# Z-Zheng/ever

Measured on AMD Instinct MI355X. Metric: 512x512 tiles/sec fwd+bwd, FarSeg-R50, higher is better.
Workload: dtype f32; 1 GPU; FarSeg ResNet-50 FPN (FarSegHead defaults, BCE+dice), 3-band 512x512, batch 16/GPU, fwd+bwd+SGD step, inputs resident in HBM; global_batch=16, parallelism=single

## Files before the change

### ever_amd/_C.py

```python
import ctypes as C
import os

_LIB_PATH = os.path.join(os.path.dirname(os.path.abspath(__file__)), 'lib', 'libever_hip.so')
_LIB_PATH = os.environ.get('EVK_LIB', _LIB_PATH)

c_void_p, c_int, c_i32, c_i64, c_u32, c_f32, c_size_t = (
    C.c_void_p, C.c_int, C.c_int32, C.c_int64, C.c_uint32, C.c_float, C.c_size_t)


class ConvDesc(C.Structure):
    _fields_ = [(n, c_i32) for n in (
        'N', 'H', 'W', 'Cin', 'Ho', 'Wo', 'Cout', 'kh', 'kw',
        'stride_h', 'stride_w', 'pad_h', 'pad_w', 'dil_h', 'dil_w')]


class SplitJob(C.Structure):
    _fields_ = [('w', c_void_p), ('out', c_void_p), ('kind', c_i32), ('arg', c_i32 * 13)]


P = c_void_p
_DP = C.POINTER(ConvDesc)
_JP = C.POINTER(SplitJob)

SIGNATURES = {
# ... 58 lines not shown
    'evk_bn_plan': (c_int, [c_i64, c_i32, c_i32, C.POINTER(c_i32)]),
    'evk_bn_fwd_train': (c_int, [P, P, P, P, P, P, c_f32, c_f32, P, P, P, c_i64, c_i32, c_u32, P, c_size_t, P, P]),
    'evk_bn_fwd_train_parts': (c_int, [P, P, P, P, P, P, c_f32, c_f32, P, P, P, c_i64, c_i32, c_u32, P, c_i32, P, c_size_t, P, P]),
    'evk_bn_fwd_train_parts_bits': (c_int, [P, P, P, P, P, P, c_f32, c_f32, P, P, P, c_i64, c_i32, c_u32, P, c_i32, P, c_size_t, P, P, P]),
    'evk_relu_bits_bytes': (c_size_t, [c_i64]),
    'evk_relu_bits_apply': (c_int, [P, P, P, c_i64, P]),
    'evk_bn_fwd_eval': (c_int, [P, P, P, P, P, P, c_f32, P, P, P, c_i64, c_i32, c_u32, P, c_size_t, P, P]),
    'evk_bn_relu_pool_fwd_train_parts': (c_int, [P, P, P, P, P, c_f32, c_f32, P, P, P, P, c_i32, c_i32, c_i32, c_i32, P, c_i32,
                                                 P, c_size_t, P, P]),
    'evk_bn_relu_pool_bwd': (c_int, [P, P, P, P, P, P, P, P, P, P, c_i32, c_i32, c_i32, c_i32, c_i32, P, c_size_t, P, P]),
    'evk_bn_bwd': (c_int, [P, P, P, P, P, P, P, P, P, P, P, c_i64, c_i32, c_u32, c_i32, P, c_size_t, P, P]),
    'evk_stream_fork': (c_int, [P, P]),
    'evk_streams_overlap': (c_int, [P, P, c_i32, P]),
    'evk_bn_relu_dot_fwd': (c_int, [P, P, P, P, P, c_i64, c_i32, c_i32, P]),
    'evk_bn_relu_dot_workspace_bytes': (c_size_t, [c_i64, c_i32, c_i32]),
    'evk_bn_relu_dot_bwd': (c_int, [P, P, P, P, P, P, P, P, P, P, P, P, c_i64, c_i32, c_i32, c_u32, P, c_size_t, P, P]),
    'evk_bn_finalize_parts': (c_int, [P, c_i32, c_i32, c_i64, P, P, P, P, c_f32, c_f32, P, P, P, P]),
    'evk_relation_bn_fwd': (c_int, [P, P, P, P, P, P, P, c_i32, c_i32, c_i32, P, P]),
    'evk_relation_bn_parts': (c_i32, [c_i32, c_i32]),
    'evk_relation_bn_workspace_bytes': (c_size_t, [c_i32, c_i32, c_i32]),
    'evk_relation_bn_bwd': (c_int, [P, P, P, P, P, P, P, P, P, P, P, P, c_i32, c_i32, c_i32, P, c_size_t, P]),
    'evk_bn_bwd_from_partials': (c_int, [P, P, P, P, P, P, P, c_i32, P, P, P, c_i64, c_i32, c_u32, c_i32, P, c_size_t, P, P]),
    'evk_bn_bwd_bits': (c_int, [P, P, P, P, P, P, P, P, P, P, P, c_i64, c_i32, c_u32, c_i32, P, c_size_t, P, P, P]),
    'evk_relu_fwd': (c_int, [P, P, c_i64, P]),
    'evk_relu_bwd': (c_int, [P, P, P, c_i64, P]),
    'evk_add': (c_int, [P, P, P, c_i64, P]),
    'evk_scale': (c_int, [P, c_f32, P, c_i64, P]),
    'evk_group_weight_expand': (c_int, [P, P, c_i32, c_i32, c_i32, c_i32, P]),
    'evk_group_weight_gather': (c_int, [P, P, c_i32, c_i32, c_i32, c_i32, P]),
    'evk_mul_scale': (c_int, [P, P, c_f32, P, c_i64, P]),
    'evk_gelu_fwd': (c_int, [P, P, c_i64, P]),
    'evk_gelu_bwd': (c_int, [P, P, P, c_i64, P]),
    'evk_maxpool3x3s2_fwd': (c_int, [P, P, P, c_i32, c_i32, c_i32, c_i32, P]),
    'evk_maxpool3x3s2_bwd': (c_int, [P, P, P, c_i32, c_i32, c_i32, c_i32, P]),
    'evk_upsample_nearest2x_add_fwd': (c_int, [P, P, P, c_i32, c_i32, c_i32, c_i32, P, P]),
    'evk_upsample_nearest2x_bwd': (c_int, [P, P, c_i32, c_i32, c_i32, c_i32, P]),
    'evk_subsample2_fwd': (c_int, [P, P, c_i32, c_i32, c_i32, c_i32, P]),
    'evk_subsample2_bwd': (c_int, [P, P, c_i32, c_i32, c_i32, c_i32, P]),
    'evk_upsample_bilinear_fwd': (c_int, [P, P, c_i32, c_i32, c_i32, c_i32, c_i32, c_i32, P]),
    'evk_upsample_bilinear_bwd': (c_int, [P, P, c_i32, c_i32, c_i32, c_i32, c_i32, c_i32, P]),
    'evk_upsample_bilinear_plan': (c_int, [c_i32, c_i32, c_i32, c_i32, c_i32, c_i32, c_i32, c_i32, C.POINTER(c_i32)]),
    'evk_upsample_bilinear_slice_fwd': (c_int, [P, P, c_i32, c_i32, c_i32, c_i32, c_i32, c_i32, c_i32, c_i32, P]),
    'evk_upsample_bilinear_slice_bwd': (c_int, [P, P, c_i32, c_i32, c_i32, c_i32, c_i32, c_i32, c_i32, c_i32, P]),
    'evk_hr_fuse_fwd': (c_int, [P, P, P, c_i32, P, P, P, c_i32, c_i32, c_i32, c_i32, P]),
    'evk_hr_fuse_bwd': (c_int, [P, P, P, P, P, P, c_i32, c_i32, c_i32, c_i32, P]),
    'evk_wfuse_fwd': (c_int, [P, P, c_i32, P, c_i32, c_f32, P, c_i32, c_i32, c_i32, c_i32, P]),
# ... 103 lines not shown
```

### ever_amd/csrc/bn.hip

```cpp
#include "bn_common.hpp"

namespace evk {

__global__ __launch_bounds__(256) void bn_stats_partial_kernel(const float* __restrict__ x, float* __restrict__ partial,
                                                               int64_t rows, int C, int64_t rows_per_blk, int tpc,
                                                               int rl) {
  __shared__ f32x4 red[2][256];
  const int c4 = C >> 2;
  const int tc = threadIdx.x % tpc, tr = threadIdx.x / tpc;
  const int64_t r0 = (int64_t)blockIdx.x * rows_per_blk;
  const int64_t r1 = min(rows, r0 + rows_per_blk);
  for (int cb = tc; cb < c4; cb += tpc) {
    f32x4 s = {0.f, 0.f, 0.f, 0.f}, q = {0.f, 0.f, 0.f, 0.f};
    const f32x4 pv = *reinterpret_cast<const f32x4*>(x + cb * 4);
    if (tr < rl) {
      int64_t r = r0 + tr;
      const int64_t st = rl;
      for (; r + 3 * st < r1; r += 4 * st) {
        const f32x4 v0 = *reinterpret_cast<const f32x4*>(x + r * C + cb * 4) - pv;
        const f32x4 v1 = *reinterpret_cast<const f32x4*>(x + (r + st) * C + cb * 4) - pv;
        const f32x4 v2 = *reinterpret_cast<const f32x4*>(x + (r + 2 * st) * C + cb * 4) - pv;
        const f32x4 v3 = *reinterpret_cast<const f32x4*>(x + (r + 3 * st) * C + cb * 4) - pv;
        s += (v0 + v1) + (v2 + v3);
        q += (v0 * v0 + v1 * v1) + (v2 * v2 + v3 * v3);
// ... 698 lines not shown
  hipLaunchKernelGGL(bn_bwd_sums_final_kernel, dim3((C + kFinCh - 1) / kFinCh), dim3(256), 0, st, (const float*)partial,
                     pl.nblk, C, sums);
  return check_launch("bn_bwd_local_sums");
}

extern "C" int evk_bn_bwd_apply_sums(const float* dy, const float* x, const float* y, const float* gamma,
                                     const float* beta, const float* mean, const float* invstd, const float* mean_g,
                                     const float* mean_gx, float* dx, int64_t rows, int32_t C, uint32_t flags,
                                     void* workspace, size_t workspace_bytes, void* stream) {
  EVK_REQUIRE(dy && x && mean && invstd && mean_g && mean_gx && dx, EVK_E_INVALID, "bn_bwd_apply_sums: null pointer");
  const int relu = (flags & EVK_BN_RELU) ? (y ? 1 : 2) : 0;
  int rc = bn_check("bn_bwd_apply_sums", rows, C, workspace, workspace_bytes, BnWorkspace::bytes(C));
  if (rc) return rc;
  hipStream_t st = (hipStream_t)stream;
  float* coef = (float*)workspace;
  hipLaunchKernelGGL(bn_bwd_coef_kernel, dim3((C + 255) / 256), dim3(256), 0, st, gamma, invstd, mean_g, mean_gx, C, coef);
  rc = check_launch("bn_bwd_coef");
  if (rc) return rc;
  const size_t n4 = (size_t)rows * C / 4;
  hipLaunchKernelGGL(bn_bwd_apply_kernel<false>, dim3(oneshot_grid(n4)), dim3(256), 0, st, dy, x, y, mean,
                     invstd, (const float*)coef, gamma, beta, dx, n4, C, relu, (uint32_t*)nullptr);
  return check_launch("bn_bwd_apply_sums");
}
```

### ever_amd/csrc/bn_common.hpp

```cpp
#pragma once
#include "x3_common.hpp"

namespace evk {

__device__ __forceinline__ unsigned bn_blk() { return gridDim.x - 1u - blockIdx.x; }

__device__ __forceinline__ int bn_fin_group() { return xcd_remap((int)blockIdx.x, (int)gridDim.x); }

__device__ __forceinline__ f32x4 bn_ld(const float* p, size_t i) {
  return __builtin_nontemporal_load(reinterpret_cast<const f32x4*>(p) + i);
}

constexpr int kMaxStatBlocks = 2048;

__device__ __forceinline__ void zero_amax(uint32_t* __restrict__ amax) {
  if (amax && blockIdx.x == 0 && threadIdx.x < kAmaxSlots) amax[threadIdx.x * kAmaxStride] = 0;
}

struct BnPlan {
  int nblk;
  int64_t rows_per_blk;
  int tpc, rl;
};
inline BnPlan bn_plan(int64_t rows, int C, int64_t per_override = 0, int64_t cap_override = 0) {
// ... 47 lines not shown
__device__ __forceinline__ f32x4 relu_mask(f32x4 g, const f32x4 yy) {
  g.x = yy.x > 0.f ? g.x : 0.f; g.y = yy.y > 0.f ? g.y : 0.f;
  g.z = yy.z > 0.f ? g.z : 0.f; g.w = yy.w > 0.f ? g.w : 0.f;
  return g;
}

__device__ __forceinline__ void fold_store_record(f32x4 (*red)[256], f32x4 s, f32x4 q, float* rec, size_t blk, int C, int cb,
                                                  int tc, int tr, int tpc, int rl) {
  red[0][threadIdx.x] = s;
  red[1][threadIdx.x] = q;
  __syncthreads();
  if (tr == 0) {
    for (int k = 1; k < rl; ++k) {
      s += red[0][k * tpc + tc];
      q += red[1][k * tpc + tc];
    }
    float* o = rec + blk * 2 * C;
    *reinterpret_cast<f32x4*>(o + cb * 4) = s;
    *reinterpret_cast<f32x4*>(o + C + cb * 4) = q;
  }
  __syncthreads();
}

constexpr int kFinCh = 8;
template <int FC, typename T, typename Op>
__device__ __forceinline__ T fold_channel_lanes(T v, T (*lds)[FC], Op op) {
#pragma unroll
  for (int o = FC; o < 64; o <<= 1) v = op(v, __shfl_xor(v, o, 64));
  const int lane = threadIdx.x & 63, w = threadIdx.x >> 6;
  if (lane < FC) lds[w][lane] = v;
  __syncthreads();
  const int tc = threadIdx.x % FC;
  const T r = op(op(lds[0][tc], lds[1][tc]), op(lds[2][tc], lds[3][tc]));
  __syncthreads();
  return r;
}
template <int FC = kFinCh>
__device__ __forceinline__ bool reduce_partials(const float* __restrict__ partial, int nblk, int C, int& c, double& s,
                                                double& q) {
  __shared__ double red[4][FC];
  const int tc = threadIdx.x % FC, tl = threadIdx.x / FC;
  c = bn_fin_group() * FC + tc;
  s = 0.0;
  q = 0.0;
  if (c < C) {
    const float* ps = partial + c;
// ... 47 lines not shown
```

### ever_amd/hip/_base.py

```python
import ctypes
import os

import torch
from torch.autograd import Function
from torch.autograd.function import once_differentiable

from .. import _C
from . import timing, weight_planes
from .workspace import workspace


class HipPathError(RuntimeError):
    """Raised when the HIP path is asked to run on something it cannot (CPU tensor, wrong dtype)."""


_CONV_MATH = os.environ.get('EVK_CONV_MATH', 'f16x2')
_MATH_MODES = ('f16x2', 'bf16x3', 'f32', 'bf16')


def _planes_math():
    return _CONV_MATH in ('f16x2', 'bf16x3', 'bf16')


def _f16x2():
# ... 114 lines not shown
    import torch.distributed as dist
    return dist.is_available() and dist.is_initialized()


def _collectives_world():
    import torch.distributed as dist
    return dist.get_world_size() if _dist_initialized() else 1


def _mark_packed(t, bits):
    _note_amax(t, bits)
    t._evk_packed = (t._version, t.data_ptr())
    absmax_stats['packed'] += 1
    return t


def _is_packed(t):
    hit = getattr(t, '_evk_packed', None)
    return hit is not None and hit[0] == t._version and hit[1] == t.data_ptr()


_RELU_BITS = os.environ.get('EVK_RELU_BITS', '1') != '0'
_LAZY_RES = os.environ.get('EVK_LAZY_RES', '1') != '0'
relu_bits_stats = {'forward': 0, 'lazy': 0, 'masked_dgrad': 0, 'masked_bn': 0, 'materialized': 0}


def _lazy_bits(t):
    hit = getattr(t, '_evk_relu_bits', None)
    if hit is not None and hit[0] == t._version and hit[1] == t.data_ptr():
        return hit[2]
    return None


def materialize_lazy(t):
    bits = _lazy_bits(t) if t is not None else None
    if bits is None:
        return t
    out = torch.empty_like(t)
    _C.call('evk_relu_bits_apply', t.data_ptr(), bits.data_ptr(), out.data_ptr(), t.numel(), _stream())
    relu_bits_stats['materialized'] += 1
    return _inherit_amax(out, t)


_top_saved_hooks = getattr(torch._C._autograd, '_top_saved_tensors_default_hooks', None)


def observers_active():
# ... 94 lines not shown
```

### ever_amd/hip/norm.py

```python
import ctypes
import os

import torch
from torch.autograd import Function
from torch.autograd.function import once_differentiable

from .. import _C
from . import timing, weight_planes
from .workspace import workspace
from ._base import (
    HipPathError, _AMAX_HANDOFF, _LAZY_RES, _PACKED, _RELU_BITS, _amax_out, _amax_zeroed, _f16x2, _inherit_amax,
    _lazy_bits, _mark_packed, _note_amax, _ptr, _require_cuda, _stream, _timed_call, as_nhwc, empty_nhwc, materialize_lazy,
    observers_active, relu_bits_stats,
)


class _BatchNormActFn(Function):

    @staticmethod
    def forward(ctx, x, residual, weight, bias, running_mean, running_var, training, momentum, eps, relu, parts=None,
                pack_out=False, lazy_res=False):
        n, c, h, w = x.shape
        rows = n * h * w
        dev = x.device
        st = _stream()
        lib = _C.load()
        ws_bytes = lib.evk_bn_workspace_bytes(rows, c)
        ws = workspace(dev, ws_bytes)
        y = empty_nhwc(n, c, h, w, dev)
        save_mean = torch.empty((c,), device=dev, dtype=torch.float32)
        save_invstd = torch.empty((c,), device=dev, dtype=torch.float32)
        flags = 1 if relu else 0
        pack = bool(pack_out and _PACKED and _f16x2() and training and parts is not None and residual is None
                    and c % 8 == 0 and rows >= 256 and not observers_active())
        abits = _amax_zeroed(dev) if pack else _amax_out(dev)
# ... 88 lines not shown
    if x.shape[1] % 4 != 0:
        raise HipPathError(f'batch_norm: channel count {x.shape[1]} must be a multiple of 4')
    if residual is not None:
        residual = as_nhwc(residual, 'batch_norm.residual')
    use_batch_stats = training or running_mean is None
    parts = getattr(x, '_evk_bn_parts', None) if use_batch_stats else None
    if parts is not None:
        del x._evk_bn_parts
    _AMAX_HANDOFF[0] = None
    if use_batch_stats and running_mean is not None:
        weight_planes.note_running_stats_changed()
    y = _BatchNormActFn.apply(x, residual, weight, bias, running_mean, running_var, bool(use_batch_stats),
                              0.0 if momentum is None else momentum, eps, bool(relu), parts, bool(pack_out), bool(lazy_res))
    if _AMAX_HANDOFF[0] is not None:
        abits, packed = _AMAX_HANDOFF[0]
        if packed:
            _mark_packed(y, abits)
        elif abits is not None:
            _note_amax(y, abits)
        _AMAX_HANDOFF[0] = None
    return y


class _BnReluPoolFn(Function):

    @staticmethod
    def forward(ctx, x, weight, bias, running_mean, running_var, momentum, eps, parts):
        n, c, h, w = x.shape
        ho, wo = (h - 1) // 2 + 1, (w - 1) // 2 + 1
        dev, st = x.device, _stream()
        ws_bytes = _C.load().evk_bn_workspace_bytes(n * h * w, c)
        ws = workspace(dev, ws_bytes)
        y = empty_nhwc(n, c, ho, wo, dev)
        code = torch.empty((n, ho, wo, c), device=dev, dtype=torch.uint8)
        save_mean = torch.empty((c,), device=dev, dtype=torch.float32)
        save_invstd = torch.empty((c,), device=dev, dtype=torch.float32)
        abits = _amax_out(dev)
        nb = 4.0 * x.numel() + 5.0 * y.numel()
        _timed_call('bn', nb, 'evk_bn_relu_pool_fwd_train_parts', x.data_ptr(), _ptr(weight), _ptr(bias), _ptr(running_mean),
                    _ptr(running_var), float(momentum), float(eps), y.data_ptr(), code.data_ptr(), save_mean.data_ptr(),
                    save_invstd.data_ptr(), n, h, w, c, parts[0].data_ptr(), parts[1], ws.data_ptr(), ws_bytes, _ptr(abits), st)
        _AMAX_HANDOFF[0] = (abits, False)
        ctx.save_for_backward(x, weight, bias, save_mean, save_invstd, code)
        ctx.mark_non_differentiable(*[t for t in (running_mean, running_var) if t is not None])
        return y

# ... 60 lines not shown
```

### ever_amd/module/_resnets.py

```python
import torch.nn as nn

from ..hip import functional as HF
from .fold import _takes_epilogue_stats, _use_folded, conv_bn
from .layers import AdaptiveAvgPool2d, BatchNorm2d, Conv2d, GroupNorm, HipSequential, MaxPool2d, ReLU

__all__ = ['ResNet', 'BasicBlock', 'Bottleneck', 'resnet18', 'resnet34', 'resnet50', 'resnet101', 'resnet152',
           'resnext50_32x4d', 'resnext101_32x4d', 'resnext101_32x8d', 'resnet50_v1c', 'resnet101_v1c']


def conv3x3(cin, cout, stride=1, groups=1, dilation=1):
    return Conv2d(cin, cout, kernel_size=3, stride=stride, padding=dilation, groups=groups, bias=False,
                  dilation=dilation)


def conv1x1(cin, cout, stride=1):
    return Conv2d(cin, cout, kernel_size=1, stride=stride, bias=False)


def _norm(norm_layer):
    if norm_layer is None or norm_layer is nn.BatchNorm2d or norm_layer is BatchNorm2d:
        return BatchNorm2d

    def make(num_features):
        m = norm_layer(num_features)
        if isinstance(m, nn.GroupNorm):
            m.__class__ = GroupNorm
        elif isinstance(m, nn.BatchNorm2d) and not isinstance(m, nn.SyncBatchNorm):
            m.__class__ = BatchNorm2d
        elif not isinstance(m, nn.SyncBatchNorm):
            raise NotImplementedError(f'ever_amd ResNet: norm layer {type(m).__name__} has no HIP kernel (BatchNorm2d, '
                                      f'SyncBatchNorm and GroupNorm are implemented)')
        return m
    return make


def _plain_norm(m):
    return not isinstance(m, BatchNorm2d)


def _norm_act(norm, x, relu):
    return norm(x, relu=relu) if isinstance(norm, GroupNorm) else (HF.relu(norm(x)) if relu else norm(x))


def _inference(bn):
    import torch
    return (not bn.training) and not torch.is_grad_enabled()


def _fork(block, x):
    if block.downsample is None:
        return HF.conv2d_fork(x, block.conv1, bn_stats=(_takes_epilogue_stats(block.bn1), False))
    h, s = HF.conv2d_fork(x, block.conv1, block.downsample[0],
                          bn_stats=(_takes_epilogue_stats(block.bn1), _takes_epilogue_stats(block.downsample[1])))
    return h, block.downsample[1](s)


def _lazy_ok(block, bn):
    from .layers import BatchNorm2d
    if type(bn) is not BatchNorm2d or bn._forward_hooks:
        return False
    mods = [block.conv1]
    ds = block.downsample
    if ds is not None:
        if len(ds) != 2 or type(ds[1]) is not BatchNorm2d:
            return False
        mods += [ds, ds[0], ds[1]]
    return not any(m._forward_hooks or m._forward_pre_hooks for m in mods)


class BasicBlock(nn.Module):
    expansion = 1

    def __init__(self, inplanes, planes, stride=1, downsample=None, groups=1, base_width=64, dilation=1,
                 norm_layer=None):
        super().__init__()
        norm_layer = _norm(norm_layer)
        if groups != 1 or base_width != 64:
            raise ValueError('BasicBlock only supports groups=1 and base_width=64')
        if dilation > 1:
            raise NotImplementedError('Dilation > 1 not supported in BasicBlock')
        self.conv1 = conv3x3(inplanes, planes, stride)
        self.bn1 = norm_layer(planes)
        self.relu = ReLU(inplace=True)
        self.conv2 = conv3x3(planes, planes)
        self.bn2 = norm_layer(planes)
        self.downsample = downsample
        self.stride = stride

    def forward(self, x):
        if _plain_norm(self.bn1):
            shortcut = x if self.downsample is None else self.downsample(x)
            out = _norm_act(self.bn1, self.conv1(x), True)
            return HF.relu(HF.add(_norm_act(self.bn2, self.conv2(out), False), shortcut))
        if _inference(self.bn1):
            shortcut = x if self.downsample is None else conv_bn(self.downsample[0], self.downsample[1], x)
            out = conv_bn(self.conv1, self.bn1, x, relu=True)
            return conv_bn(self.conv2, self.bn2, out, residual=shortcut, relu=True)
        h, shortcut = _fork(self, x)
        out = self.bn1(h, relu=True, conv_only=True)
        return conv_bn(self.conv2, self.bn2, out, residual=shortcut, relu=True, lazy_res=_lazy_ok(self, self.bn2))


class Bottleneck(nn.Module):
    expansion = 4

    def __init__(self, inplanes, planes, stride=1, downsample=None, groups=1, base_width=64, dilation=1,
                 norm_layer=None):
        super().__init__()
        norm_layer = _norm(norm_layer)
        width = int(planes * (base_width / 64.)) * groups
        self.conv1 = conv1x1(inplanes, width)
        self.bn1 = norm_layer(width)
        self.conv2 = conv3x3(width, width, stride, groups, dilation)
        self.bn2 = norm_layer(width)
        self.conv3 = conv1x1(width, planes * self.expansion)
        self.bn3 = norm_layer(planes * self.expansion)
        self.relu = ReLU(inplace=True)
        self.downsample = downsample
        self.stride = stride

    def forward(self, x):
        if _plain_norm(self.bn1):
            shortcut = x if self.downsample is None else self.downsample(x)
            out = _norm_act(self.bn1, self.conv1(x), True)
            out = _norm_act(self.bn2, self.conv2(out), True)
            return HF.relu(HF.add(_norm_act(self.bn3, self.conv3(out), False), shortcut))
        if _inference(self.bn1):
            shortcut = x if self.downsample is None else conv_bn(self.downsample[0], self.downsample[1], x)
            out = conv_bn(self.conv1, self.bn1, x, relu=True)
            out = conv_bn(self.conv2, self.bn2, out, relu=True)
            return conv_bn(self.conv3, self.bn3, out, residual=shortcut, relu=True)
        h, shortcut = _fork(self, x)
        out = self.bn1(h, relu=True, conv_only=True)
        out = conv_bn(self.conv2, self.bn2, out, relu=True, conv_only=True)
        return conv_bn(self.conv3, self.bn3, out, residual=shortcut, relu=True, lazy_res=_lazy_ok(self, self.bn3))


class ResNet(nn.Module):
    def __init__(self, block, layers, num_classes=1000, zero_init_residual=False, groups=1, width_per_group=64,
                 replace_stride_with_dilation=None, norm_layer=None, deep_stem=False):
        super().__init__()
        norm_layer = _norm(norm_layer)
        self._norm_layer = norm_layer
        self.inplanes = 64
        self.dilation = 1
        if replace_stride_with_dilation is None:
            replace_stride_with_dilation = [False, False, False]
        if len(replace_stride_with_dilation) != 3:
            raise ValueError('replace_stride_with_dilation should be None or a 3-element tuple, got {}'.format(
                replace_stride_with_dilation))
        self.groups = groups
        self.base_width = width_per_group
        self.deep_stem = deep_stem
        if deep_stem:
            half = self.inplanes // 2
            self.stem = HipSequential(
                Conv2d(3, half, 3, 2, 1, bias=False), BatchNorm2d(half), ReLU(inplace=True),
                Conv2d(half, half, 3, 1, 1, bias=False), BatchNorm2d(half), ReLU(inplace=True),
# ... 130 lines not shown
```

### ever_amd/module/layers.py

```python
import torch
import torch.nn as nn

from ..hip import functional as HF

__all__ = ['Conv2d', 'ConvTranspose2d', 'BatchNorm2d', 'ReLU', 'MaxPool2d', 'UpsamplingBilinear2d', 'UpsamplingNearest2d', 'AdaptiveAvgPool2d',
           'Identity', 'Dropout', 'GELU', 'HipSequential', 'run_sequence', 'to_hip']

Identity = nn.Identity


class Conv2d(nn.Conv2d):

    def __init__(self, *args, **kwargs):
        super().__init__(*args, **kwargs)
        _check_conv(self)
        self.weight.data = self.weight.data.contiguous(memory_format=torch.channels_last)

    def forward(self, x, relu=False, bn_stats=False):
        if self.groups != 1 and HF.depthwise_in_scope(self.in_channels, self.out_channels, self.groups, self.kernel_size,
                                                      self.stride, self.dilation):
            return HF.depthwise_conv2d(x, self.weight, self.bias, self.stride, self.padding, self.dilation, relu=relu)
        w = self.weight if self.groups == 1 else HF.grouped_dense_weight(self.weight, self.groups)
        y = HF.conv2d(x, w, self.bias, self.stride, self.padding, self.dilation, relu=relu, bn_stats=bn_stats)
        if self._forward_hooks and getattr(y, '_evk_bn_parts', None) is not None and len(y._evk_bn_parts) > 2:
# ... 43 lines not shown
    def forward_relu_pool(self, x):
        training = self.training or (self.running_mean is None)
        if not training or self.momentum is None:
            return HF.max_pool3x3s2(self.forward(x, relu=True))
        if self.training and self.track_running_stats and self.num_batches_tracked is not None:
            self._nbt_pending = getattr(self, '_nbt_pending', 0) + 1
        rm = self.running_mean if self.track_running_stats else None
        rv = self.running_var if self.track_running_stats else None
        return HF.batch_norm_relu_max_pool(x, self.weight, self.bias, rm, rv, self.momentum, self.eps)

    def flush_num_batches_tracked(self):
        pending = getattr(self, '_nbt_pending', 0)
        if pending and self.num_batches_tracked is not None:
            self.num_batches_tracked.add_(pending)
        self._nbt_pending = 0

    def _save_to_state_dict(self, destination, prefix, keep_vars):
        self.flush_num_batches_tracked()
        super()._save_to_state_dict(destination, prefix, keep_vars)

    def _load_from_state_dict(self, *args, **kwargs):
        self._nbt_pending = 0
        super()._load_from_state_dict(*args, **kwargs)


class ReLU(nn.ReLU):
    def forward(self, x):
        return HF.relu(x)


class MaxPool2d(nn.MaxPool2d):

    def forward(self, x):
        cfg = (_one(self.kernel_size), _one(self.stride), _one(self.padding), _one(self.dilation), self.ceil_mode)
        if cfg != (3, 2, 1, 1, False):
            raise NotImplementedError(f'ever_amd MaxPool2d: only (k=3,s=2,p=1) is implemented, got {cfg}')
        return HF.max_pool3x3s2(x)


def _one(v):
    if isinstance(v, (tuple, list)):
        if len(set(v)) != 1:
            return tuple(v)
        return v[0]
    return v

# ... 117 lines not shown
```

### include/ever_hip.h

```cpp
#ifndef EVER_HIP_H_
#define EVER_HIP_H_

#include <stddef.h>
#include <stdint.h>

#ifdef __cplusplus
extern "C" {
#endif

#define EVK_OK 0
#define EVK_E_INVALID (-1)
#define EVK_E_UNSUPPORTED (-2)
#define EVK_E_LAUNCH (-3)
#define EVK_E_WORKSPACE (-4)

const char* evk_last_error(void);
int evk_abi_version(void);
const char* evk_build_arch(void);

typedef struct evk_conv_desc {
  int32_t N, H, W, Cin;
  int32_t Ho, Wo, Cout;
  int32_t kh, kw;
  int32_t stride_h, stride_w;
// ... 139 lines not shown
int evk_relu_bits_apply(const float* g, const uint32_t* bits, float* out, int64_t n, void* stream);
int evk_bn_relu_pool_fwd_train_parts(const float* x, const float* gamma, const float* beta, float* running_mean,
                                     float* running_var, float momentum, float eps, float* y, uint8_t* code,
                                     float* save_mean, float* save_invstd, int32_t N, int32_t H, int32_t W, int32_t C,
                                     const float* parts, int32_t nparts, void* workspace, size_t workspace_bytes,
                                     uint32_t* y_absmax, void* stream);
int evk_bn_relu_pool_bwd(const float* dp, const uint8_t* code, const float* x, const float* gamma, const float* beta,
                         const float* save_mean, const float* save_invstd, float* dx, float* dgamma, float* dbeta,
                         int32_t N, int32_t H, int32_t W, int32_t C, int32_t train, void* workspace,
                         size_t workspace_bytes, uint32_t* dx_absmax, void* stream);
int evk_bn_fwd_eval(const float* x, const float* residual, const float* gamma, const float* beta,
                    const float* running_mean, const float* running_var, float eps, float* y,
                    float* save_mean , float* save_invstd ,
                    int64_t rows, int32_t C, uint32_t flags, void* workspace, size_t workspace_bytes,
                    uint32_t* y_absmax, void* stream);
int evk_bn_bwd(const float* dy, const float* x, const float* y, const float* gamma, const float* beta,
               const float* save_mean, const float* save_invstd, float* dx, float* d_residual,
               float* dgamma, float* dbeta, int64_t rows, int32_t C, uint32_t flags, int32_t train,
               void* workspace, size_t workspace_bytes, uint32_t* dx_absmax, void* stream);
int evk_bn_bwd_bits(const float* dy, const float* x, const float* y, const float* gamma, const float* beta,
                    const float* save_mean, const float* save_invstd, float* dx, float* d_residual,
                    float* dgamma, float* dbeta, int64_t rows, int32_t C, uint32_t flags, int32_t train,
                    void* workspace, size_t workspace_bytes, uint32_t* dx_absmax, const uint32_t* relu_bits, void* stream);

int evk_stream_fork(void* from, void* to);

int evk_streams_overlap(void* a, void* b, int32_t us, float* elapsed_us);

int evk_relu_fwd(const float* x, float* y, int64_t n, void* stream);
int evk_relu_bwd(const float* dy, const float* y, float* dx, int64_t n, void* stream);
int evk_add(const float* a, const float* b, float* out, int64_t n, void* stream);
int evk_scale(const float* a, float alpha, float* out, int64_t n, void* stream);
int evk_group_weight_expand(const float* w, float* dense, int32_t Cout, int32_t taps, int32_t Cin, int32_t groups, void* stream);
int evk_group_weight_gather(const float* ddense, float* dw, int32_t Cout, int32_t taps, int32_t Cin, int32_t groups, void* stream);
int evk_mul_scale(const float* a, const float* b, float alpha, float* out, int64_t n, void* stream);
int evk_gelu_fwd(const float* x, float* y, int64_t n, void* stream);
int evk_gelu_bwd(const float* dy, const float* x, float* dx, int64_t n, void* stream);

int evk_maxpool3x3s2_fwd(const float* x, float* y, uint8_t* code, int32_t N, int32_t H, int32_t W,
                         int32_t C, void* stream);
int evk_maxpool3x3s2_bwd(const float* dy, const uint8_t* code, float* dx, int32_t N, int32_t H,
                         int32_t W, int32_t C, void* stream);

int evk_upsample_nearest2x_add_fwd(const float* top, const float* lateral, float* out, int32_t N,
                                   int32_t H, int32_t W, int32_t C, uint32_t* out_absmax, void* stream);
int evk_upsample_nearest2x_bwd(const float* dout, float* dtop, int32_t N, int32_t H, int32_t W,
// ... 193 lines not shown
```

Measured before the change: 566.7 tiles/s.

## Fuse main-branch and downsample BatchNorm with residual add and ReLU in blocks

In downsample ResNet blocks, the shortcut BN and the final BN+residual+ReLU now run as one paired kernel set. The forward pass normalizes both conv outputs, adds them, applies ReLU and writes relu bits in a single elementwise pass, so the normalized shortcut tensor is never materialized. The backward pass computes both BNs' reduction partials in one sweep over dy and apply-phase dx for both branches in one kernel. This removes an intermediate activation write/read and several launches per downsample block, at the cost of more fallback logic and extra reduction state.

```diff
diff --git a/ever_amd/_C.py b/ever_amd/_C.py
--- a/ever_amd/_C.py
+++ b/ever_amd/_C.py
@@ -104,6 +104,9 @@
     'evk_relation_bn_bwd': (c_int, [P, P, P, P, P, P, P, P, P, P, P, P, c_i32, c_i32, c_i32, P, c_size_t, P]),
     'evk_bn_bwd_from_partials': (c_int, [P, P, P, P, P, P, P, c_i32, P, P, P, c_i64, c_i32, c_u32, c_i32, P, c_size_t, P, P]),
     'evk_bn_bwd_bits': (c_int, [P, P, P, P, P, P, P, P, P, P, P, c_i64, c_i32, c_u32, c_i32, P, c_size_t, P, P, P]),
+    'evk_bn_pair_fwd_train_parts_bits': (c_int, [P, P, P, P, P, P, c_f32, c_f32, P, P, P, P, c_f32, c_f32, P, P, P, P, P, c_i64, c_i32,
+                                                 P, c_i32, P, c_i32, P, c_size_t, P, P, P]),
+    'evk_bn_pair_bwd_bits': (c_int, [P, P, P, P, P, P, P, P, P, P, P, P, P, P, P, c_i64, c_i32, c_u32, c_u32, P, c_size_t, P, P, P, P]),
     'evk_relu_fwd': (c_int, [P, P, c_i64, P]),
     'evk_relu_bwd': (c_int, [P, P, P, c_i64, P]),
     'evk_add': (c_int, [P, P, P, c_i64, P]),
diff --git a/ever_amd/csrc/bn.hip b/ever_amd/csrc/bn.hip
--- a/ever_amd/csrc/bn.hip
+++ b/ever_amd/csrc/bn.hip
@@ -744,3 +744,233 @@
                      invstd, (const float*)coef, gamma, beta, dx, n4, C, relu, (uint32_t*)nullptr);
   return check_launch("bn_bwd_apply_sums");
 }
+
+namespace evk {
+
+__global__ __launch_bounds__(256) void bn_pair_apply_kernel(const float* __restrict__ x3, const float* __restrict__ xs,
+                                                            const float* __restrict__ ss3, const float* __restrict__ sss,
+                                                            float* __restrict__ y, size_t n4, int C,
+                                                            uint32_t* __restrict__ amax, uint32_t* __restrict__ relu_bits) {
+  const size_t base = (size_t)bn_blk() * 256;
+  const size_t i = base + threadIdx.x;
+  const bool valid = i < n4;
+  f32x4 v = {0.f, 0.f, 0.f, 0.f};
+  if (valid) {
+    const int c4 = C >> 2;
+    const int cb = chunk_of(base, c4);
+    const f32x4 sc3 = reinterpret_cast<const f32x4*>(ss3)[cb];
+    const f32x4 sh3 = reinterpret_cast<const f32x4*>(ss3 + C)[cb];
+    const f32x4 scs = reinterpret_cast<const f32x4*>(sss)[cb];
+    const f32x4 shs = reinterpret_cast<const f32x4*>(sss + C)[cb];
+    v = bn_ld(x3, i) * sc3 + sh3;
+    const f32x4 xv = bn_ld(xs, i);
+    f32x4 s;
+    s.x = __builtin_fmaf(xv.x, scs.x, shs.x); s.y = __builtin_fmaf(xv.y, scs.y, shs.y);
+    s.z = __builtin_fmaf(xv.z, scs.z, shs.z); s.w = __builtin_fmaf(xv.w, scs.w, shs.w);
+    v += s;
+  }
+  if ((i & ~(size_t)63) < n4) relu_bits_store(relu_bits, i >> 6, v.x > 0.f, v.y > 0.f, v.z > 0.f, v.w > 0.f);
+  if (valid) {
+    v.x = fmaxf(v.x, 0.f); v.y = fmaxf(v.y, 0.f); v.z = fmaxf(v.z, 0.f); v.w = fmaxf(v.w, 0.f);
+    reinterpret_cast<f32x4*>(y)[i] = v;
+  }
+  if (amax) block_absmax(v, valid, amax);
+}
+
+template <bool PK3, bool PKS>
+__global__ __launch_bounds__(256) void bn_pair_bwd_partial_kernel(
+    const float* __restrict__ dy, const float* __restrict__ x3, const float* __restrict__ xs,
+    const float* __restrict__ mean3, const float* __restrict__ invstd3, const float* __restrict__ means,
+    const float* __restrict__ invstds, float* __restrict__ partial3, float* __restrict__ partials, int64_t rows, int C,
+    int64_t rows_per_blk, int tpc, int rl, float* __restrict__ pmax3, float* __restrict__ pmaxs,
+    const uint32_t* __restrict__ bits) {
+  __shared__ f32x4 red[2][256];
+  const int c4 = C >> 2;
+  const int tc = threadIdx.x % tpc, tr = threadIdx.x / tpc;
+  const int64_t r0 = (int64_t)bn_blk() * rows_per_blk;
+  const int64_t r1 = min(rows, r0 + rows_per_blk);
+  for (int cb = tc; cb < c4; cb += tpc) {
+    const f32x4 mu3 = *reinterpret_cast<const f32x4*>(mean3 + cb * 4);
+    const f32x4 is3 = *reinterpret_cast<const f32x4*>(invstd3 + cb * 4);
+    const f32x4 mus = *reinterpret_cast<const f32x4*>(means + cb * 4);
+    const f32x4 iss = *reinterpret_cast<const f32x4*>(invstds + cb * 4);
+    f32x4 s = {0.f, 0.f, 0.f, 0.f}, q3 = {0.f, 0.f, 0.f, 0.f}, qs = {0.f, 0.f, 0.f, 0.f};
+    f32x4 gm = {0.f, 0.f, 0.f, 0.f}, xm3 = {0.f, 0.f, 0.f, 0.f}, xms = {0.f, 0.f, 0.f, 0.f};
+    if (tr < rl) {
+      auto one = [&](const f32x4 gin, const f32x4 xv3, const f32x4 xvs, size_t off) {
+        const f32x4 g = relu_bits_mask(gin, bits, off >> 2);
+        s += g;
+        const f32x4 xh3 = (xv3 - mu3) * is3;
+        q3 += g * xh3;
+        const f32x4 xhs = (xvs - mus) * iss;
+        qs += g * xhs;
+        if constexpr (PK3 || PKS) {
+          gm.x = fmaxf(gm.x, fabsf(g.x)); gm.y = fmaxf(gm.y, fabsf(g.y));
+          gm.z = fmaxf(gm.z, fabsf(g.z)); gm.w = fmaxf(gm.w, fabsf(g.w));
+        }
+        if constexpr (PK3) {
+          xm3.x = fmaxf(xm3.x, fabsf(xh3.x)); xm3.y = fmaxf(xm3.y, fabsf(xh3.y));
+          xm3.z = fmaxf(xm3.z, fabsf(xh3.z)); xm3.w = fmaxf(xm3.w, fabsf(xh3.w));
+        }
+        if constexpr (PKS) {
+          xms.x = fmaxf(xms.x, fabsf(xhs.x)); xms.y = fmaxf(xms.y, fabsf(xhs.y));
+          xms.z = fmaxf(xms.z, fabsf(xhs.z)); xms.w = fmaxf(xms.w, fabsf(xhs.w));
+        }
+      };
+      int64_t r = r0 + tr;
+      const int64_t st = rl;
+      for (; r + 3 * st < r1; r += 4 * st) {
+        const size_t o0 = (size_t)r * C + cb * 4, o1 = (size_t)(r + st) * C + cb * 4;
+        const size_t o2 = (size_t)(r + 2 * st) * C + cb * 4, o3 = (size_t)(r + 3 * st) * C + cb * 4;
+        const f32x4 g0 = bp_ld(dy + o0), g1 = bp_ld(dy + o1);
+        const f32x4 g2 = bp_ld(dy + o2), g3 = bp_ld(dy + o3);
+        const f32x4 a0 = bp_ld(x3 + o0), a1 = bp_ld(x3 + o1);
+        const f32x4 a2 = bp_ld(x3 + o2), a3 = bp_ld(x3 + o3);
+        const f32x4 b0 = bp_ld(xs + o0), b1 = bp_ld(xs + o1);
+        const f32x4 b2 = bp_ld(xs + o2), b3 = bp_ld(xs + o3);
+        one(g0, a0, b0, o0);
+        one(g1, a1, b1, o1);
+        one(g2, a2, b2, o2);
+        one(g3, a3, b3, o3);
+      }
+      for (; r < r1; r += st) {
+        const size_t o0 = (size_t)r * C + cb * 4;
+        const f32x4 g0 = bp_ld(dy + o0);
+        const f32x4 a0 = bp_ld(x3 + o0);
+        const f32x4 b0 = bp_ld(xs + o0);
+        one(g0, a0, b0, o0);
+      }
+    }
+    fold_store_record(red, s, q3, partial3, bn_blk(), C, cb, tc, tr, tpc, rl);
+    fold_store_record(red, s, qs, partials, bn_blk(), C, cb, tc, tr, tpc, rl);
+    if constexpr (PK3) fold_store_maxima(red, gm, xm3, pmax3, bn_blk(), C, cb, tc, tr, tpc, rl);
+    if constexpr (PKS) fold_store_maxima(red, gm, xms, pmaxs, bn_blk(), C, cb, tc, tr, tpc, rl);
+  }
+}
+
+template <bool PK3, bool PKS>
+__global__ __launch_bounds__(256) void bn_pair_bwd_apply_kernel(
+    const float* __restrict__ dy, const float* __restrict__ x3, const float* __restrict__ xs,
+    const float* __restrict__ mean3, const float* __restrict__ invstd3, const float* __restrict__ coef3,
+    const float* __restrict__ means, const float* __restrict__ invstds, const float* __restrict__ coefs,
+    float* __restrict__ dx3, float* __restrict__ dxs, size_t n4, int C, uint32_t* __restrict__ amax3,
+    uint32_t* __restrict__ amaxs, const uint32_t* __restrict__ bits) {
+  const size_t base = (size_t)bn_blk() * 256;
+  const size_t i = base + threadIdx.x;
+  const bool valid = i < n4;
+  f32x4 out3 = {0.f, 0.f, 0.f, 0.f}, outs = {0.f, 0.f, 0.f, 0.f};
+  float pk_inv3 = 1.f, pk_invs = 1.f;
+  if constexpr (PK3) pk_inv3 = op_scale(amax3[0]).inv;
+  if constexpr (PKS) pk_invs = op_scale(amaxs[0]).inv;
+  if (valid) {
+    const int c4 = C >> 2;
+    const int c = chunk_of(base, c4);
+    const f32x4 g = relu_bits_mask(bn_ld(dy, i), bits, i);
+    {
+      const f32x4 k0 = reinterpret_cast<const f32x4*>(coef3)[c];
+      const f32x4 k1 = reinterpret_cast<const f32x4*>(coef3 + C)[c];
+      const f32x4 k2 = reinterpret_cast<const f32x4*>(coef3 + 2 * C)[c];
+      const f32x4 mu = reinterpret_cast<const f32x4*>(mean3)[c];
+      const f32x4 is = reinterpret_cast<const f32x4*>(invstd3)[c];
+      const f32x4 xh = (bn_ld(x3, i) - mu) * is;
+      out3 = k0 * (g - k1 - xh * k2);
+      if constexpr (PK3) {
+        reinterpret_cast<u32x4*>(dx3)[i] = pack_hl4(out3, pk_inv3);
+      } else {
+        reinterpret_cast<f32x4*>(dx3)[i] = out3;
+      }
+    }
+    {
+      const f32x4 k0 = reinterpret_cast<const f32x4*>(coefs)[c];
+      const f32x4 k1 = reinterpret_cast<const f32x4*>(coefs + C)[c];
+      const f32x4 k2 = reinterpret_cast<const f32x4*>(coefs + 2 * C)[c];
+      const f32x4 mu = reinterpret_cast<const f32x4*>(means)[c];
+      const f32x4 is = reinterpret_cast<const f32x4*>(invstds)[c];
+      const f32x4 xh = (bn_ld(xs, i) - mu) * is;
+      outs = k0 * (g - k1 - xh * k2);
+      if constexpr (PKS) {
+        reinterpret_cast<u32x4*>(dxs)[i] = pack_hl4(outs, pk_invs);
+      } else {
+        reinterpret_cast<f32x4*>(dxs)[i] = outs;
+      }
+    }
+  }
+  if constexpr (!PK3)
+    if (amax3) block_absmax(out3, valid, amax3);
+  if constexpr (!PK3 && !PKS) __syncthreads();
+  if constexpr (!PKS)
+    if (amaxs) block_absmax(outs, valid, amaxs);
+}
+
+#define EVK_BN_LAUNCH_PK2(kernel, pk3, pks, grid, st, ...)                                             \
+  do {                                                                                                \
+    if (pk3 && pks) hipLaunchKernelGGL((kernel<true, true>), grid, dim3(256), 0, st, __VA_ARGS__);     \
+    else if (pk3) hipLaunchKernelGGL((kernel<true, false>), grid, dim3(256), 0, st, __VA_ARGS__);      \
+    else if (pks) hipLaunchKernelGGL((kernel<false, true>), grid, dim3(256), 0, st, __VA_ARGS__);      \
+    else hipLaunchKernelGGL((kernel<false, false>), grid, dim3(256), 0, st, __VA_ARGS__);              \
+  } while (0)
+
+}
+
+extern "C" int evk_bn_pair_fwd_train_parts_bits(
+    const float* x3, const float* xs, const float* gamma3, const float* beta3, float* running_mean3, float* running_var3,
+    float momentum3, float eps3, const float* gammas, const float* betas, float* running_means, float* running_vars,
+    float momentums, float epss, float* y, float* save_mean3, float* save_invstd3, float* save_means, float* save_invstds,
+    int64_t rows, int32_t C, const float* parts3, int32_t nparts3, const float* partss, int32_t npartss, void* workspace,
+    size_t workspace_bytes, uint32_t* y_absmax, uint32_t* relu_bits, void* stream) {
+  EVK_REQUIRE(x3 && xs && y && save_mean3 && save_invstd3 && save_means && save_invstds && parts3 && nparts3 > 0 && partss &&
+                  npartss > 0 && relu_bits,
+              EVK_E_INVALID, "bn_pair_fwd_train_parts_bits: bad argument");
+  int rc = bn_check("bn_pair_fwd_train_parts_bits", rows, C, workspace, workspace_bytes, 2 * BnWorkspace::bytes(C));
+  if (rc) return rc;
+  hipStream_t st = (hipStream_t)stream;
+  float* ss3 = BnWorkspace(workspace, C).coef;
+  float* sss = BnWorkspace((char*)workspace + BnWorkspace::bytes(C), C).coef;
+  launch_parts_final(st, parts3, nparts3, C, (double)rows, gamma3, beta3, running_mean3, running_var3, momentum3, eps3,
+                     save_mean3, save_invstd3, ss3, y_absmax, 0);
+  rc = check_launch("bn_parts_final");
+  if (rc) return rc;
+  launch_parts_final(st, partss, npartss, C, (double)rows, gammas, betas, running_means, running_vars, momentums, epss,
+                     save_means, save_invstds, sss, nullptr, 0);
+  rc = check_launch("bn_parts_final");
+  if (rc) return rc;
+  const size_t n4 = (size_t)rows * C / 4;
+  hipLaunchKernelGGL(bn_pair_apply_kernel, dim3(oneshot_grid(n4)), dim3(256), 0, st, x3, xs, (const float*)ss3,
+                     (const float*)sss, y, n4, C, y_absmax, relu_bits);
+  return check_launch("bn_pair_apply");
+}
+
+extern "C" int evk_bn_pair_bwd_bits(const float* dy, const float* x3, const float* xs, const float* gamma3,
+                                    const float* gammas, const float* save_mean3, const float* save_invstd3,
+                                    const float* save_means, const float* save_invstds, float* dx3, float* dxs, float* dgamma3,
+                                    float* dbeta3, float* dgammas, float* dbetas, int64_t rows, int32_t C, uint32_t flags3,
+                                    uint32_t flagss, void* workspace, size_t workspace_bytes, uint32_t* dx3_absmax,
+                                    uint32_t* dxs_absmax, const uint32_t* relu_bits, void* stream) {
+  EVK_REQUIRE(dy && x3 && xs && save_mean3 && save_invstd3 && save_means && save_invstds && dx3 && dxs && relu_bits,
+              EVK_E_INVALID, "bn_pair_bwd_bits: null pointer");
+  int rc = bn_check("bn_pair_bwd_bits", rows, C, workspace, workspace_bytes, 2 * BnWorkspace::bytes(C));
+  if (rc) return rc;
+  const bool pk3 = (flags3 & EVK_BN_PACK_DX) != 0, pks = (flagss & EVK_BN_PACK_DX) != 0;
+  EVK_REQUIRE((!pk3 || dx3_absmax) && (!pks || dxs_absmax), EVK_E_INVALID,
+              "bn_pair_bwd_bits: EVK_BN_PACK_DX needs that dx's absmax buffer (slots zero on entry)");
+  hipStream_t st = (hipStream_t)stream;
+  const BnPlan pl = bn_plan(rows, C);
+  const BnWorkspace w3(workspace, C), wss((char*)workspace + BnWorkspace::bytes(C), C);
+  float* pmax3 = pk3 ? w3.pmax : nullptr;
+  float* pmaxs = pks ? wss.pmax : nullptr;
+  EVK_BN_LAUNCH_PK2(bn_pair_bwd_partial_kernel, pk3, pks, dim3(pl.nblk), st, dy, x3, xs, save_mean3, save_invstd3, save_means,
+                    save_invstds, w3.partial, wss.partial, rows, C, pl.rows_per_blk, pl.tpc, pl.rl, pmax3, pmaxs, relu_bits);
+  rc = check_launch("bn_pair_bwd_partial");
+  if (rc) return rc;
+  launch_bn_bwd_final(st, w3.partial, pl.nblk, C, rows, gamma3, save_invstd3, dgamma3, dbeta3, w3.coef, 1, dx3_absmax, pmax3);
+  rc = check_launch("bn_bwd_final");
+  if (rc) return rc;
+  launch_bn_bwd_final(st, wss.partial, pl.nblk, C, rows, gammas, save_invstds, dgammas, dbetas, wss.coef, 1, dxs_absmax, pmaxs);
+  rc = check_launch("bn_bwd_final");
+  if (rc) return rc;
+  const size_t n4 = (size_t)rows * C / 4;
+  EVK_BN_LAUNCH_PK2(bn_pair_bwd_apply_kernel, pk3, pks, dim3(oneshot_grid(n4)), st, dy, x3, xs, save_mean3, save_invstd3,
+                    (const float*)w3.coef, save_means, save_invstds, (const float*)wss.coef, dx3, dxs, n4, C, dx3_absmax,
+                    dxs_absmax, relu_bits);
+  return check_launch("bn_pair_bwd_apply");
+}
diff --git a/ever_amd/csrc/bn_common.hpp b/ever_amd/csrc/bn_common.hpp
--- a/ever_amd/csrc/bn_common.hpp
+++ b/ever_amd/csrc/bn_common.hpp
@@ -93,6 +93,24 @@
   __syncthreads();
 }
 
+__device__ __forceinline__ void fold_store_maxima(f32x4 (*red)[256], f32x4 gm, f32x4 xm, float* pm, size_t blk, int C, int cb,
+                                                  int tc, int tr, int tpc, int rl) {
+  red[0][threadIdx.x] = gm;
+  red[1][threadIdx.x] = xm;
+  __syncthreads();
+  if (tr == 0) {
+    for (int k = 1; k < rl; ++k) {
+      const f32x4 a = red[0][k * tpc + tc], b = red[1][k * tpc + tc];
+      gm.x = fmaxf(gm.x, a.x); gm.y = fmaxf(gm.y, a.y); gm.z = fmaxf(gm.z, a.z); gm.w = fmaxf(gm.w, a.w);
+      xm.x = fmaxf(xm.x, b.x); xm.y = fmaxf(xm.y, b.y); xm.z = fmaxf(xm.z, b.z); xm.w = fmaxf(xm.w, b.w);
+    }
+    float* o = pm + blk * 2 * C;
+    *reinterpret_cast<f32x4*>(o + cb * 4) = gm;
+    *reinterpret_cast<f32x4*>(o + C + cb * 4) = xm;
+  }
+  __syncthreads();
+}
+
 constexpr int kFinCh = 8;
 template <int FC, typename T, typename Op>
 __device__ __forceinline__ T fold_channel_lanes(T v, T (*lds)[FC], Op op) {
diff --git a/ever_amd/hip/_base.py b/ever_amd/hip/_base.py
--- a/ever_amd/hip/_base.py
+++ b/ever_amd/hip/_base.py
@@ -160,7 +160,8 @@
 
 _RELU_BITS = os.environ.get('EVK_RELU_BITS', '1') != '0'
 _LAZY_RES = os.environ.get('EVK_LAZY_RES', '1') != '0'
-relu_bits_stats = {'forward': 0, 'lazy': 0, 'masked_dgrad': 0, 'masked_bn': 0, 'materialized': 0}
+_BN_PAIR = os.environ.get('EVK_BN_PAIR', '1') != '0'
+relu_bits_stats = {'forward': 0, 'lazy': 0, 'masked_dgrad': 0, 'masked_bn': 0, 'materialized': 0, 'pair': 0}
 
 
 def _lazy_bits(t):
diff --git a/ever_amd/hip/norm.py b/ever_amd/hip/norm.py
--- a/ever_amd/hip/norm.py
+++ b/ever_amd/hip/norm.py
@@ -9,8 +9,9 @@
 from . import timing, weight_planes
 from .workspace import workspace
 from ._base import (
-    HipPathError, _AMAX_HANDOFF, _LAZY_RES, _PACKED, _RELU_BITS, _amax_out, _amax_zeroed, _f16x2, _inherit_amax,
-    _lazy_bits, _mark_packed, _note_amax, _ptr, _require_cuda, _stream, _timed_call, as_nhwc, empty_nhwc, materialize_lazy,
+    HipPathError, _AMAX_HANDOFF, _BN_PAIR, _LAZY_RES, _PACKED, _RELU_BITS, _amax_out, _amax_zeroed, _f16x2, _inherit_amax,
+    _lazy_bits, _mark_packed, _note_amax, _ptr, _require_cuda, _stream, _timed_call, as_nhwc, empty_nhwc, is_nhwc,
+    materialize_lazy,
     observers_active, relu_bits_stats,
 )
 
@@ -145,6 +146,96 @@
     return y
 
 
+class _BnPairActFn(Function):
+
+    @staticmethod
+    def forward(ctx, x3, xs, w3, b3, ws_, bs, rm3, rv3, rms, rvs, mom3, eps3, moms, epss, parts3, partss):
+        n, c, h, w = x3.shape
+        rows = n * h * w
+        dev = x3.device
+        st = _stream()
+        lib = _C.load()
+        ws_bytes = 2 * lib.evk_bn_workspace_bytes(rows, c)
+        ws = workspace(dev, ws_bytes)
+        y = empty_nhwc(n, c, h, w, dev)
+        sm3, si3, sms, sis = (torch.empty((c,), device=dev, dtype=torch.float32) for _ in range(4))
+        abits = _amax_out(dev)
+        rbits = torch.empty((lib.evk_relu_bits_bytes(x3.numel()) // 4,), device=dev, dtype=torch.int32)
+        relu_bits_stats['forward'] += 1
+        relu_bits_stats['pair'] += 1
+        _timed_call('bn', 4.0 * x3.numel() * 3, 'evk_bn_pair_fwd_train_parts_bits', x3.data_ptr(), xs.data_ptr(), _ptr(w3), _ptr(b3),
+                    _ptr(rm3), _ptr(rv3), float(mom3), float(eps3), _ptr(ws_), _ptr(bs), _ptr(rms), _ptr(rvs), float(moms),
+                    float(epss), y.data_ptr(), sm3.data_ptr(), si3.data_ptr(), sms.data_ptr(), sis.data_ptr(), rows, c,
+                    parts3[0].data_ptr(), parts3[1], partss[0].data_ptr(), partss[1], ws.data_ptr(), ws_bytes, _ptr(abits),
+                    rbits.data_ptr(), st)
+        _AMAX_HANDOFF[0] = (abits, False)
+        ctx.pack_dx3 = bool(len(parts3) > 2 and parts3[2])
+        ctx.pack_dxs = bool(len(partss) > 2 and partss[2])
+        ctx.save_for_backward(x3, xs, w3, ws_, sm3, si3, sms, sis, rbits)
+        ctx.mark_non_differentiable(*[t for t in (rm3, rv3, rms, rvs) if t is not None])
+        return y
+
+    @staticmethod
+    @once_differentiable
+    def backward(ctx, dy):
+        x3, xs, w3, ws_, sm3, si3, sms, sis, rbits = ctx.saved_tensors
+        n, c, h, w = x3.shape
+        rows = n * h * w
+        dev = x3.device
+        st = _stream()
+        dy = as_nhwc(materialize_lazy(dy), 'batch_norm_pair.backward')
+        lib = _C.load()
+        ws_bytes = 2 * lib.evk_bn_workspace_bytes(rows, c)
+        ws = workspace(dev, ws_bytes)
+        dx3, dxs = torch.empty_like(x3), torch.empty_like(xs)
+        dg3, db3 = ((torch.empty((c,), device=dev, dtype=torch.float32) for _ in range(2)) if w3 is not None else (None, None))
+        dgs, dbs = ((torch.empty((c,), device=dev, dtype=torch.float32) for _ in range(2)) if ws_ is not None else (None, None))
+        pack3 = ctx.pack_dx3 and _f16x2()
+        abits3 = _amax_zeroed(dev) if pack3 else _amax_out(dev)
+        pack3 = pack3 and abits3 is not None
+        packs = ctx.pack_dxs and _f16x2()
+        abitss = _amax_zeroed(dev) if packs else _amax_out(dev)
+        packs = packs and abitss is not None
+        relu_bits_stats['lazy'] += 1
+        relu_bits_stats['masked_bn'] += 1
+        _timed_call('bn', 4.0 * x3.numel() * 8, 'evk_bn_pair_bwd_bits', dy.data_ptr(), x3.data_ptr(), xs.data_ptr(), _ptr(w3),
+                    _ptr(ws_), sm3.data_ptr(), si3.data_ptr(), sms.data_ptr(), sis.data_ptr(), dx3.data_ptr(), dxs.data_ptr(),
+                    _ptr(dg3), _ptr(db3), _ptr(dgs), _ptr(dbs), rows, c, 2 if pack3 else 0, 2 if packs else 0, ws.data_ptr(),
+                    ws_bytes, _ptr(abits3), _ptr(abitss), rbits.data_ptr(), st)
+        for dx, pack, abits in ((dx3, pack3, abits3), (dxs, packs, abitss)):
+            if pack:
+                _mark_packed(dx, abits)
+            elif abits is not None:
+                _note_amax(dx, abits)
+        need = ctx.needs_input_grad
+        return (dx3, dxs, dg3 if need[2] else None, db3 if need[3] else None, dgs if need[4] else None,
+                dbs if need[5] else None) + (None,) * 10
+
+
+def bn_pair_enabled():
+    return bool(_BN_PAIR and _RELU_BITS and _LAZY_RES and not observers_active())
+
+
+def batch_norm_pair_act(x3, xs, bn3, bns):
+    if not (x3.is_cuda and xs.is_cuda and x3.shape == xs.shape and x3.dim() == 4 and x3.shape[1] % 4 == 0
+            and is_nhwc(x3) and is_nhwc(xs)):
+        return None
+    parts3, partss = getattr(x3, '_evk_bn_parts', None), getattr(xs, '_evk_bn_parts', None)
+    if parts3 is None or partss is None:
+        return None
+    del x3._evk_bn_parts, xs._evk_bn_parts
+    _AMAX_HANDOFF[0] = None
+    if bn3[2] is not None or bns[2] is not None:
+        weight_planes.note_running_stats_changed()
+    y = _BnPairActFn.apply(x3, xs, bn3[0], bn3[1], bns[0], bns[1], bn3[2], bn3[3], bns[2], bns[3], bn3[4], bn3[5], bns[4],
+                           bns[5], parts3, partss)
+    if _AMAX_HANDOFF[0] is not None:
+        if _AMAX_HANDOFF[0][0] is not None:
+            _note_amax(y, _AMAX_HANDOFF[0][0])
+        _AMAX_HANDOFF[0] = None
+    return y
+
+
 class _BnReluPoolFn(Function):
 
     @staticmethod
diff --git a/ever_amd/module/_resnets.py b/ever_amd/module/_resnets.py
--- a/ever_amd/module/_resnets.py
+++ b/ever_amd/module/_resnets.py
@@ -2,7 +2,8 @@
 
 from ..hip import functional as HF
 from .fold import _takes_epilogue_stats, _use_folded, conv_bn
-from .layers import AdaptiveAvgPool2d, BatchNorm2d, Conv2d, GroupNorm, HipSequential, MaxPool2d, ReLU
+from .layers import (AdaptiveAvgPool2d, BatchNorm2d, Conv2d, GroupNorm, HipSequential, MaxPool2d, ReLU,
+                     batch_norm_pair)
 
 __all__ = ['ResNet', 'BasicBlock', 'Bottleneck', 'resnet18', 'resnet34', 'resnet50', 'resnet101', 'resnet152',
            'resnext50_32x4d', 'resnext101_32x4d', 'resnext101_32x8d', 'resnet50_v1c', 'resnet101_v1c']
@@ -47,12 +48,12 @@
     return (not bn.training) and not torch.is_grad_enabled()
 
 
-def _fork(block, x):
+def _fork(block, x, pair=False):
     if block.downsample is None:
         return HF.conv2d_fork(x, block.conv1, bn_stats=(_takes_epilogue_stats(block.bn1), False))
     h, s = HF.conv2d_fork(x, block.conv1, block.downsample[0],
                           bn_stats=(_takes_epilogue_stats(block.bn1), _takes_epilogue_stats(block.downsample[1])))
-    return h, block.downsample[1](s)
+    return h, (s if pair else block.downsample[1](s))
 
 
 def _lazy_ok(block, bn):
@@ -66,6 +67,27 @@
             return False
         mods += [ds, ds[0], ds[1]]
     return not any(m._forward_hooks or m._forward_pre_hooks for m in mods)
+
+
+def _pair_ok(block, bn):
+    ds = block.downsample
+    if ds is None or not _lazy_ok(block, bn) or not HF.bn_pair_enabled():
+        return False
+    for m in (bn, ds[1]):
+        if not (m.training and _takes_epilogue_stats(m)) or m.momentum is None:
+            return False
+    return not any(getattr(m, h, None) for m in (bn, ds, ds[1])
+                   for h in ('_forward_hooks', '_forward_pre_hooks', '_backward_hooks', '_backward_pre_hooks'))
+
+
+def _block_end(block, conv, bn, out, shortcut, pair):
+    if not pair:
+        return conv_bn(conv, bn, out, residual=shortcut, relu=True, lazy_res=_lazy_ok(block, bn))
+    x3 = conv(out, bn_stats=True)
+    y = batch_norm_pair(bn, block.downsample[1], x3, shortcut)
+    if y is not None:
+        return y
+    return bn(x3, residual=block.downsample[1](shortcut), relu=True, lazy_res=True)
 
 
 class BasicBlock(nn.Module):
@@ -96,9 +118,10 @@
             shortcut = x if self.downsample is None else conv_bn(self.downsample[0], self.downsample[1], x)
             out = conv_bn(self.conv1, self.bn1, x, relu=True)
             return conv_bn(self.conv2, self.bn2, out, residual=shortcut, relu=True)
-        h, shortcut = _fork(self, x)
+        pair = _pair_ok(self, self.bn2)
+        h, shortcut = _fork(self, x, pair)
         out = self.bn1(h, relu=True, conv_only=True)
-        return conv_bn(self.conv2, self.bn2, out, residual=shortcut, relu=True, lazy_res=_lazy_ok(self, self.bn2))
+        return _block_end(self, self.conv2, self.bn2, out, shortcut, pair)
 
 
 class Bottleneck(nn.Module):
@@ -130,10 +153,11 @@
             out = conv_bn(self.conv1, self.bn1, x, relu=True)
             out = conv_bn(self.conv2, self.bn2, out, relu=True)
             return conv_bn(self.conv3, self.bn3, out, residual=shortcut, relu=True)
-        h, shortcut = _fork(self, x)
+        pair = _pair_ok(self, self.bn3)
+        h, shortcut = _fork(self, x, pair)
         out = self.bn1(h, relu=True, conv_only=True)
         out = conv_bn(self.conv2, self.bn2, out, relu=True, conv_only=True)
-        return conv_bn(self.conv3, self.bn3, out, residual=shortcut, relu=True, lazy_res=_lazy_ok(self, self.bn3))
+        return _block_end(self, self.conv3, self.bn3, out, shortcut, pair)
 
 
 class ResNet(nn.Module):
diff --git a/ever_amd/module/layers.py b/ever_amd/module/layers.py
--- a/ever_amd/module/layers.py
+++ b/ever_amd/module/layers.py
@@ -89,6 +89,22 @@
     def _load_from_state_dict(self, *args, **kwargs):
         self._nbt_pending = 0
         super()._load_from_state_dict(*args, **kwargs)
+
+
+def batch_norm_pair(bn, bn_short, x3, xs):
+    if x3.dim() != 4 or x3.shape[0] * x3.shape[2] * x3.shape[3] <= 1:
+        return None
+
+    def args(m):
+        track = m.track_running_stats
+        return (m.weight, m.bias, m.running_mean if track else None, m.running_var if track else None, m.momentum, m.eps)
+    y = HF.batch_norm_pair_act(x3, xs, args(bn), args(bn_short))
+    if y is None:
+        return None
+    for m in (bn, bn_short):
+        if m.track_running_stats and m.num_batches_tracked is not None:
+            m._nbt_pending = getattr(m, '_nbt_pending', 0) + 1
+    return y
 
 
 class ReLU(nn.ReLU):
diff --git a/include/ever_hip.h b/include/ever_hip.h
--- a/include/ever_hip.h
+++ b/include/ever_hip.h
@@ -185,6 +185,19 @@
                     const float* save_mean, const float* save_invstd, float* dx, float* d_residual,
                     float* dgamma, float* dbeta, int64_t rows, int32_t C, uint32_t flags, int32_t train,
                     void* workspace, size_t workspace_bytes, uint32_t* dx_absmax, const uint32_t* relu_bits, void* stream);
+int evk_bn_pair_fwd_train_parts_bits(const float* x3, const float* xs, const float* gamma3, const float* beta3,
+                                     float* running_mean3, float* running_var3, float momentum3, float eps3,
+                                     const float* gammas, const float* betas, float* running_means, float* running_vars,
+                                     float momentums, float epss, float* y, float* save_mean3, float* save_invstd3,
+                                     float* save_means, float* save_invstds, int64_t rows, int32_t C, const float* parts3,
+                                     int32_t nparts3, const float* partss, int32_t npartss, void* workspace,
+                                     size_t workspace_bytes, uint32_t* y_absmax, uint32_t* relu_bits, void* stream);
+int evk_bn_pair_bwd_bits(const float* dy, const float* x3, const float* xs, const float* gamma3, const float* gammas,
+                         const float* save_mean3, const float* save_invstd3, const float* save_means,
+                         const float* save_invstds, float* dx3, float* dxs, float* dgamma3, float* dbeta3, float* dgammas,
+                         float* dbetas, int64_t rows, int32_t C, uint32_t flags3, uint32_t flagss, void* workspace,
+                         size_t workspace_bytes, uint32_t* dx3_absmax, uint32_t* dxs_absmax, const uint32_t* relu_bits,
+                         void* stream);
 
 int evk_stream_fork(void* from, void* to);
 
```

Result: faster. 573.7 tiles/s, median of 6 (+1.2%).
